# wagnva/semantic-nerf-for-satellite-data

Measured on AMD Instinct MI355X. Metric: train rays/sec (4096 rays x 64 samples), higher is better.
Workload: dtype f32(f16x2)

## Files before the change

semantic-nerf-for-satellite-data_amd/csrc/api.hip:

```cpp
#include <stdarg.h>
#include <stdio.h>
#include <stdlib.h>
#include <string.h>

#include <mutex>

#include "aux_kernels.h"
#include "bsp.h"
#include "composite.h"
#include "gemm.h"
#include "plan.h"

namespace snerf {

int forward_bsp(const Plan& p, const float* pk, const SnerfInputs* in, const SnerfOutputs* out, void* workspace, hipStream_t st);
int backward_bsp(const Plan& p, const float* pk, const SnerfInputs* in, const SnerfOutGrads* go, float* gp, float* d_t, float* d_t_s,
                 void* workspace, hipStream_t st);

static thread_local char g_err[512] = "";
void set_error(const char* fmt, ...) {
  va_list ap;
  va_start(ap, fmt);
  vsnprintf(g_err, sizeof(g_err), fmt, ap);
  va_end(ap);
// ... 359 lines not shown
  return p.packed_floats;
}

size_t snerf_grad_floats(const SnerfDesc* desc) {
  Plan p;
  if (make_plan(desc, &p)) return 0;
  return p.n_fp32;
}

size_t snerf_workspace_bytes(const SnerfDesc* desc) {
  Plan p;
  if (make_plan(desc, &p)) return 0;
  return p.ws_bytes;
}

int snerf_pack_params(const SnerfDesc* desc, const SnerfParams* params, float* packed, void* stream) {
  Plan p;
  RC(make_plan(desc, &p));
  if (!params || !packed) { set_error("null params/packed"); return SNERF_ERR_NULL; }
  TableBuilder tb;
  build_tables(p, params, tb);
  if (tb.missing) { set_error("snerf_pack_params: a parameter tensor required by this SnerfDesc is NULL"); return SNERF_ERR_NULL; }
  hipStream_t st = (hipStream_t)stream;
  RC(launch_zero_bytes(packed, p.n_fp32 * sizeof(float), st));
  for (int i = 0; i < tb.nt; ++i) RC(launch_copy_table(tb.tabs[i], packed, 0, st));
  char* planes = reinterpret_cast<char*>(packed + p.n_fp32);
  int* exps = reinterpret_cast<int*>(planes + p.wp_bytes);
  unsigned* maxbits = reinterpret_cast<unsigned*>(exps + bsp::WPACK_MAX);
  note_plan(packed, p.compose_feats);
  if (!p.compose_feats) return bsp::launch_wpack(p.wj, packed, planes, exps, maxbits, p.pl, st);
  {
    bsp::SgTable tb;
    bsp::compose_jobs(tb, packed + p.w_h1, packed + p.w_fs, packed + p.b_fs, packed + p.b_h1, packed + p.o_wc, packed + p.o_bc, p.W, p.FA, p.N1);
    RC(bsp::launch_sgemm(tb, 64, st));
  }
  bsp::WPackTable first, rest;
  first.n = rest.n = 0;
  for (int i = 0; i < p.wj.n; ++i) (i < p.wj_first ? first.j[first.n++] : rest.j[rest.n++]) = p.wj.j[i];
  RC(bsp::launch_wpack(first, packed, planes, exps, maxbits, p.pl, st));
  return bsp::launch_wpack(rest, packed, planes, exps, maxbits, p.pl, st);
}

int snerf_unpack_grads(const SnerfDesc* desc, const float* packed_grads, const SnerfParams* grads, int accumulate,
                       void* stream) {
  Plan p;
  RC(make_plan(desc, &p));
  if (!grads || !packed_grads) { set_error("null grads"); return SNERF_ERR_NULL; }
  TableBuilder tb;
  build_tables(p, grads, tb);
  if (tb.missing) { set_error("snerf_unpack_grads: a gradient tensor required by this SnerfDesc is NULL"); return SNERF_ERR_NULL; }
  hipStream_t st = (hipStream_t)stream;
  for (int i = 0; i < tb.nt; ++i) RC(launch_copy_table(tb.tabs[i], const_cast<float*>(packed_grads), accumulate ? 2 : 1, st));
  return SNERF_OK;
}

int snerf_forward(const SnerfDesc* desc, const float* packed_params, const SnerfInputs* in, const SnerfOutputs* out,
                  void* workspace, size_t workspace_bytes, void* stream) {
  Plan p;
  RC(make_plan(desc, &p));
  if (!packed_params || !out || !workspace) { set_error("snerf_forward: null argument"); return SNERF_ERR_NULL; }
  if (workspace_bytes < p.ws_bytes) { set_error("snerf_forward: workspace too small (%zu < %zu)", workspace_bytes, p.ws_bytes); return SNERF_ERR_WORKSPACE; }
  if (((uintptr_t)workspace & 255) || ((uintptr_t)packed_params & 255)) { set_error("workspace and packed params must be 256-byte aligned"); return SNERF_ERR_WORKSPACE; }
  RC(check_inputs(p, in));
  RC(check_plan_note(packed_params, p.compose_feats, "snerf_forward", "packed parameter buffer"));
  if (p.relight) {
    RC(check_plan_note(workspace, p.compose_feats, "snerf_forward", "workspace"));
    RC(check_relight_note(workspace, desc, out->beta != nullptr));
// ... 42 lines not shown
```

semantic-nerf-for-satellite-data_amd/csrc/bsp.h:

```cpp
#pragma once
#include "common.h"
#include "gemm.h"

namespace snerf {
namespace bsp {

constexpr int RB = 128;
constexpr int CB = 128;
constexpr int E_MAX = 100;
constexpr int E_QUIET = 60;

typedef __amdgpu_buffer_rsrc_t srd_t;
typedef unsigned int u32x4 __attribute__((ext_vector_type(4)));
typedef unsigned int u32x2 __attribute__((ext_vector_type(2)));
typedef _Float16 f16x8 __attribute__((ext_vector_type(8)));
typedef _Float16 f16x4 __attribute__((ext_vector_type(4)));
constexpr unsigned OOB = 0xFFFFFFF0u;

__host__ __device__ inline int ncb_of(int ld) { return (ld + CB - 1) / CB; }
__host__ __device__ inline size_t plane_bytes(size_t rows, int ld, int pl = 2) { return rows * (size_t)ld * 2 * pl; }
__host__ __device__ inline size_t etab_ints(size_t rows, int ld) { return ((rows + RB - 1) / RB) * (size_t)ncb_of(ld); }
__host__ __device__ inline unsigned g16_off(int k, int pl = 2) { return (unsigned)(k >> 4) * 32u * (unsigned)pl + (unsigned)(k & 15) * 2u; }

__host__ __device__ inline int exp_of_maxbits(unsigned b) {
// ... 127 lines not shown
bool trunk_fusion_enabled();

int launch_kc(const KcArgs& a, hipStream_t st);
void kc_set_grid_override(int n);
int launch_kc_narrow(const KcArgs& a, hipStream_t st);
int launch_dw(const DwArgs& a, bool narrow_i, hipStream_t st);

int launch_to_planes(const float* src, int ld_src, int rows, int cols, char* dst, int* E, int ld, int col0, int pl, hipStream_t st);
int launch_from_planes(const char* src, const int* E, int ld, int col0, int rows, int cols, float* dst, int ld_dst, int pl, hipStream_t st);

struct WPackJob {
  unsigned long long src_off;
  int src_ld;
  int rows, K;
  int transposed;
  unsigned long long dst_off;
  int e_idx;
  int m_rows, m_cols;
};
constexpr int WPACK_MAX = 48;
struct WPackTable { WPackJob j[WPACK_MAX]; int n; };
constexpr int WPACK_CHUNK = 24;
struct WPackChunk { WPackJob j[WPACK_CHUNK]; int n; };
__host__ __device__ inline size_t wp16_bytes(int rows, int K, int pl = 2) { return (size_t)((rows + 31) / 32) * (size_t)(K / 16) * 1024 * pl; }
int launch_wpack(const WPackTable& tb, const float* master, char* planes, int* exps, unsigned* maxbits, int pl, hipStream_t st);

struct SgJob {
  const float* A = nullptr; long long sa_i = 0, sa_k = 0;
  const float* B = nullptr; long long sb_k = 0, sb_j = 0;
  const float* D = nullptr; int ldd = 0;
  const float* u = nullptr; const float* v = nullptr;
  float* C = nullptr; int ldc = 0;
  int M = 0, N = 0, K = 0, acc = 0;
  int blk0 = 0;
};
constexpr int SG_MAX = 6;
struct SgTable { SgJob j[SG_MAX]; int n = 0; };
int launch_sgemm(const SgTable& tb, int tile_m, hipStream_t st);
void compose_jobs(SgTable& tb, const float* w_h1, const float* w_f, const float* b_f, const float* b_h1, float* wc, float* bc, int W, int FA, int N1);
void uncompose_jobs(SgTable& tb, const float* G, const float* gc, const float* w_h1, const float* w_f, const float* b_f,
                    float* dw_h1, float* db_h1, float* dw_f, float* db_f, int W, int FA, int M);

}
struct EncodeArgs;
namespace bsp {
int launch_encode_bsp(const EncodeArgs& a, char* pe, int* Epe, char* fa, int* Efa, int fa_col0, int pl, hipStream_t st);
int launch_relight_extras(const EncodeArgs& a, char* fa, int* Efa, int fa_col0, int pl, hipStream_t st);
int launch_zero_cols(char* base, size_t pitch, size_t width_bytes, int rows, hipStream_t st);
int launch_colsum32_bsp(const float* in, int rows, float* partial, char* planes, int* E, int pl, hipStream_t st);

}
}
```

semantic-nerf-for-satellite-data_amd/csrc/bsp_aux.hip:

```cpp
#include "bsp.h"
#include "aux_kernels.h"

namespace snerf {
namespace bsp {

__device__ __forceinline__ float block_max_256(float m, float* sm) {
#pragma unroll
  for (int o = 32; o >= 1; o >>= 1) m = fmaxf(m, __shfl_xor(m, o, 64));
  __syncthreads();
  if ((threadIdx.x & 63) == 0) sm[threadIdx.x >> 6] = m;
  __syncthreads();
  return fmaxf(fmaxf(sm[0], sm[1]), fmaxf(sm[2], sm[3]));
}

__global__ __launch_bounds__(256) void to_planes_kernel(const float* __restrict__ src, int ld_src, int rows, int cols,
                                                        char* __restrict__ dst, int* __restrict__ E, int ld, int col0, int pl) {
  __shared__ float sm[4];
  const int rb = blockIdx.y, cb = blockIdx.x;
  const int t = threadIdx.x, c8 = cb * 128 + (t & 15) * 8;
  float v[8][8];
  float m = 0.f;
#pragma unroll
  for (int i = 0; i < 8; ++i) {
    const int r = rb * 128 + (t >> 4) + 16 * i;
// ... 76 lines not shown
    const int r = threadIdx.x >> 3, kp = (threadIdx.x & 7) * 2;
    const int ra = ub * 32 + wf16_row(r), ka = ks * 16 + kp;
    float x[2];
#pragma unroll
    for (int q = 0; q < 2; ++q) {
      const int k = ka + q;
      const bool ok = j.transposed ? (k < j.m_rows && ra < j.m_cols) : (ra < j.m_rows && k < j.m_cols);
      x[q] = ok ? master[j.src_off + (j.transposed ? (size_t)k * j.src_ld + ra : (size_t)ra * j.src_ld + k)] : 0.f;
    }
    const _Float16 h0 = (_Float16)(x[0] * sc), h1 = (_Float16)(x[1] * sc);
    const _Float16 l0 = (_Float16)(x[0] * sc - (float)h0), l1 = (_Float16)(x[1] * sc - (float)h1);
    typedef _Float16 f16x2 __attribute__((ext_vector_type(2)));
    char* u = planes + j.dst_off + (size_t)unit * 1024 * pl + (32 * (kp >> 3) + r) * 16 + (kp & 7) * 2;
    *reinterpret_cast<f16x2*>(u) = f16x2{h0, h1};
    if (pl == 2) *reinterpret_cast<f16x2*>(u + 1024) = f16x2{l0, l1};
  }
}

int launch_wpack(const WPackTable& tb, const float* master, char* planes, int* exps, unsigned* maxbits, int pl, hipStream_t st) {
  if (tb.n <= 0) return SNERF_OK;
  { int rc = launch_zero_bytes(maxbits, WPACK_MAX * sizeof(unsigned), st); if (rc) return rc; }
  for (int pass = 0; pass < 2; ++pass)
    for (int first = 0; first < tb.n; first += WPACK_CHUNK) {
      WPackChunk c;
      c.n = tb.n - first < WPACK_CHUNK ? tb.n - first : WPACK_CHUNK;
      for (int i = 0; i < c.n; ++i) c.j[i] = tb.j[first + i];
      if (pass == 0) hipLaunchKernelGGL(wmax_kernel, dim3(32, c.n), dim3(256), 0, st, c, master, maxbits);
      else hipLaunchKernelGGL(wpack_kernel, dim3(128, c.n), dim3(256), 0, st, c, master, planes, exps, maxbits, pl);
      SNERF_LAUNCH_CHECK();
    }
  return SNERF_OK;
}

template <int TM>
__global__ __launch_bounds__(256) void sgemm_jobs_kernel(const SgTable tb) {
  constexpr int BM = 16 * TM, BN = 64, BK = 16;
  __shared__ float As[BK][BM + 1];
  __shared__ float Bs[BK][BN + 4];
  int q = 0;
  while (q + 1 < tb.n && (int)blockIdx.x >= tb.j[q + 1].blk0) ++q;
  const SgJob jb = tb.j[q];
  const int tiles_n = (jb.N + BN - 1) / BN;
  const int tile = (int)blockIdx.x - jb.blk0;
  const int i0 = (tile / tiles_n) * BM, j0 = (tile % tiles_n) * BN;
  const int t = threadIdx.x, ty = t >> 4, tx = t & 15;
  float acc[TM][4];
#pragma unroll
  for (int r = 0; r < TM; ++r)
#pragma unroll
    for (int c = 0; c < 4; ++c) acc[r][c] = 0.f;
  const bool a_k_fast = jb.sa_k == 1, b_j_fast = jb.sb_j == 1;
  for (int k0 = 0; k0 < jb.K; k0 += BK) {
#pragma unroll
    for (int s = 0; s < (BM * BK) / 256; ++s) {
      const int idx = t + 256 * s;
      const int i = a_k_fast ? idx / BK : idx % BM, k = a_k_fast ? idx % BK : idx / BM;
      As[k][i] = (i0 + i < jb.M && k0 + k < jb.K) ? jb.A[(long long)(i0 + i) * jb.sa_i + (long long)(k0 + k) * jb.sa_k] : 0.f;
    }
#pragma unroll
    for (int s = 0; s < (BN * BK) / 256; ++s) {
      const int idx = t + 256 * s;
      const int j = b_j_fast ? idx % BN : idx / BK, k = b_j_fast ? idx / BN : idx % BK;
      Bs[k][j] = (j0 + j < jb.N && k0 + k < jb.K) ? jb.B[(long long)(k0 + k) * jb.sb_k + (long long)(j0 + j) * jb.sb_j] : 0.f;
    }
    __syncthreads();
#pragma unroll
    for (int k = 0; k < BK; ++k) {
      float a[TM], b[4];
#pragma unroll
      for (int r = 0; r < TM; ++r) a[r] = As[k][ty * TM + r];
#pragma unroll
      for (int c = 0; c < 4; ++c) b[c] = Bs[k][tx * 4 + c];
#pragma unroll
      for (int r = 0; r < TM; ++r)
#pragma unroll
        for (int c = 0; c < 4; ++c) acc[r][c] = fmaf(a[r], b[c], acc[r][c]);
    }
    __syncthreads();
  }
#pragma unroll
  for (int r = 0; r < TM; ++r) {
    const int i = i0 + ty * TM + r;
    if (i >= jb.M) continue;
#pragma unroll
    for (int c = 0; c < 4; ++c) {
      const int j = j0 + tx * 4 + c;
      if (j >= jb.N) continue;
      float x = acc[r][c];
      if (jb.u) x = fmaf(jb.u[i], jb.v[j], x);
      if (jb.D) x += jb.D[(size_t)i * jb.ldd + j];
      float* o = jb.C + (size_t)i * jb.ldc + j;
      *o = jb.acc ? *o + x : x;
    }
  }
}

void compose_jobs(SgTable& tb, const float* w_h1, const float* w_f, const float* b_f, const float* b_h1, float* wc, float* bc, int W, int FA, int N1) {
  const int X = FA - W;
  tb.n = 0;
  auto job = [&]() -> SgJob& { tb.j[tb.n] = SgJob(); return tb.j[tb.n++]; };
  { SgJob& j = job(); j.A = w_h1; j.sa_i = FA; j.sa_k = 1; j.B = w_f; j.sb_k = W; j.sb_j = 1; j.C = wc; j.ldc = FA; j.M = N1; j.N = W; j.K = W; }
  { SgJob& j = job(); j.D = w_h1 + W; j.ldd = FA; j.C = wc + W; j.ldc = FA; j.M = N1; j.N = X; }
  { SgJob& j = job(); j.D = w_f + (size_t)W * W; j.ldd = W; j.C = wc + (size_t)N1 * FA; j.ldc = FA; j.M = 32; j.N = W; }
  { SgJob& j = job(); j.C = wc + (size_t)N1 * FA + W; j.ldc = FA; j.M = 32; j.N = X; }
  { SgJob& j = job(); j.A = w_h1; j.sa_i = FA; j.sa_k = 1; j.B = b_f; j.sb_k = 1; j.sb_j = 0; j.D = b_h1; j.ldd = 1; j.C = bc; j.ldc = 1; j.M = N1; j.N = 1; j.K = W; }
}
void uncompose_jobs(SgTable& tb, const float* G, const float* gc, const float* w_h1, const float* w_f, const float* b_f,
                    float* dw_h1, float* db_h1, float* dw_f, float* db_f, int W, int FA, int M) {
  tb.n = 0;
  auto job = [&]() -> SgJob& { tb.j[tb.n] = SgJob(); return tb.j[tb.n++]; };
  { SgJob& j = job(); j.A = G; j.sa_i = FA; j.sa_k = 1; j.B = w_f; j.sb_k = 1; j.sb_j = W; j.u = gc; j.v = b_f; j.C = dw_h1; j.ldc = FA; j.M = M; j.N = W; j.K = W; j.acc = 1; }
  { SgJob& j = job(); j.A = w_h1; j.sa_i = 1; j.sa_k = FA; j.B = G; j.sb_k = FA; j.sb_j = 1; j.C = dw_f; j.ldc = W; j.M = W; j.N = W; j.K = M; j.acc = 1; }
  { SgJob& j = job(); j.A = w_h1; j.sa_i = 1; j.sa_k = FA; j.B = gc; j.sb_k = 1; j.sb_j = 0; j.C = db_f; j.ldc = 1; j.M = W; j.N = 1; j.K = M; j.acc = 1; }
  { SgJob& j = job(); j.D = gc; j.ldd = 1; j.C = db_h1; j.ldc = 1; j.M = M; j.N = 1; j.acc = 1; }
}

int launch_sgemm(const SgTable& tb0, int tile_m, hipStream_t st) {
  if (tb0.n <= 0) return SNERF_OK;
  if (tb0.n > SG_MAX || (tile_m != 64 && tile_m != 32)) { set_error("sgemm: bad job table"); return SNERF_ERR_BAD_DESC; }
  SgTable tb = tb0;
  int blocks = 0;
  for (int q = 0; q < tb.n; ++q) {
    SgJob& j = tb.j[q];
    if (!j.C || j.M <= 0 || j.N <= 0 || j.K < 0 || j.ldc < 1 || (j.K > 0 && (!j.A || !j.B)) || (j.u && !j.v) || (j.D && j.ldd < 1)) {
      set_error("sgemm: bad job %d", q);
      return SNERF_ERR_BAD_DESC;
    }
    j.blk0 = blocks;
    blocks += ((j.M + tile_m - 1) / tile_m) * ((j.N + 63) / 64);
  }
  if (tile_m == 64) hipLaunchKernelGGL(sgemm_jobs_kernel<4>, dim3(blocks), dim3(256), 0, st, tb);
  else hipLaunchKernelGGL(sgemm_jobs_kernel<2>, dim3(blocks), dim3(256), 0, st, tb);
  SNERF_LAUNCH_CHECK();
  return SNERF_OK;
}

__global__ void zero_cols_kernel(char* base, size_t pitch, int width16, int rows) {
  const int i = blockIdx.x * blockDim.x + threadIdx.x;
  if (i >= rows * width16) return;
  const int r = i / width16, c = i - r * width16;
  *reinterpret_cast<u32x4*>(base + (size_t)r * pitch + 16 * (size_t)c) = u32x4{0u, 0u, 0u, 0u};
}
int launch_zero_cols(char* base, size_t pitch, size_t width_bytes, int rows, hipStream_t st) {
  const int w16 = (int)(width_bytes / 16);
  if (w16 <= 0 || rows <= 0) return SNERF_OK;
  hipLaunchKernelGGL(zero_cols_kernel, dim3((unsigned)(((size_t)rows * w16 + 255) / 256)), dim3(256), 0, st, base, pitch, w16, rows);
  SNERF_LAUNCH_CHECK();
  return SNERF_OK;
}

__device__ __forceinline__ void point_xyz(const EncodeArgs& a, long long point, float (&x)[3]) {
  const int n = (int)((unsigned)point / (unsigned)a.S);
#pragma unroll
  for (int c = 0; c < 3; ++c) {
    if (a.xyz != nullptr) {
      x[c] = a.xyz[point * 3 + c];
    } else {
#pragma clang fp contract(off)
      const float o = a.rays[n * 8 + c];
      const float d = a.dir_is_sun ? a.sun_d[(size_t)n * a.sun_stride + c] : a.rays[n * 8 + 3 + c];
      const float dz = d * a.z[point];
      x[c] = o + dz;
    }
  }
}
// ... 197 lines not shown
```

semantic-nerf-for-satellite-data_amd/csrc/bsp_gemm.hip:

```cpp
#include "bsp_dev.h"

#include <vector>

namespace snerf {
namespace bsp {

constexpr int KC_STRIP = 32 * 68 * 4;
constexpr int KN_A = 128 * 64, KN_RING = 4, KN_TAIL = KN_RING * KN_A, KN_LDS = KN_TAIL + 512;

template <int PL>
__global__ __launch_bounds__(256, 4) void gemm_kcn_kernel(const KcArgs p) {
  constexpr int EB = 2 * PL, KSUB = PL == 2 ? 16 : 32, KSH = PL == 2 ? 4 : 5;
  __shared__ __attribute__((aligned(16))) char lds[KN_LDS];
  int* etab = reinterpret_cast<int*>(lds + KN_TAIL);
  const int t = threadIdx.x, lane = t & 63;
  const int wave = __builtin_amdgcn_readfirstlane(t >> 6);
  const int ti = blockIdx.x, i0 = ti * 128, wi0 = wave * 32;
  const int nks16 = p.K >> 4;
  const int nks = (p.K + KSUB - 1) >> KSH, nks1 = nks;
  const srd_t srdA = make_srd(p.A + ((size_t)i0 * p.lda + p.a_col0) * EB,
                              clamp_bytes(i0 < p.I ? ((unsigned long long)(p.I - i0 - 1) * p.lda + p.Ka) * (unsigned long long)EB : 0ull));
  const srd_t srdW = make_srd(p.W, p.w_bytes);
  unsigned voA[2];
#pragma unroll
  for (int q = 0; q < 2; ++q) {
    const int row = 64 * q + (t >> 2);
    const unsigned c = (unsigned)((t & 3) ^ ((row >> 2) & 3));
    voA[q] = (i0 + row < p.I) ? (unsigned)row * (unsigned)p.lda * (unsigned)EB + 16u * c : OOB;
  }
  const unsigned w_u0 = (unsigned)(p.w_row0 >> 5), w_ks0 = (unsigned)(p.w_k0 >> 4);
  auto issueA = [&](int s, int slot) {
#pragma unroll
    for (int q = 0; q < 2; ++q) dma16(srdA, lds + slot * KN_A + 4096 * q + wave * 1024, s < nks ? voA[q] : OOB, (unsigned)s * 64u);
  };
// ... 29 lines not shown
  const unsigned fo0 = (unsigned)rowl * 64u + (unsigned)(((0 + kh) ^ swz) << 4);
  const unsigned fo1 = (unsigned)rowl * 64u + (unsigned)(((2 + kh) ^ swz) << 4);
  auto step = [&](int s, int slot, BFrag& bc, BFrag& bn) {
    wait_vm<2>();
    barrier_raw();
    if (__builtin_expect(((s < 64 ? chg0 >> s : chg1 >> (s - 64)) & 1ull) != 0ull, 0)) acc = scale_acc(acc, etab[s] - etab[s - 1]);
    loadB(s + 1, bn);
    issueA(s + 2, (slot + 2) % KN_RING);
    const char* st = lds + slot * KN_A;
    if constexpr (PL == 2) {
      acc = mfma3(ldsfrag(st + wi0 * 64 + fo0), ldsfrag(st + wi0 * 64 + fo1), __builtin_bit_cast(f16x8, bc.h), __builtin_bit_cast(f16x8, bc.l), acc);
    } else {
      acc = __builtin_amdgcn_mfma_f32_32x32x16_f16(ldsfrag(st + wi0 * 64 + fo0), __builtin_bit_cast(f16x8, bc.h), acc, 0, 0, 0);
      acc = __builtin_amdgcn_mfma_f32_32x32x16_f16(ldsfrag(st + wi0 * 64 + fo1), __builtin_bit_cast(f16x8, bc.l), acc, 0, 0, 0);
    }
  };
  for (int s = 0; s < nks; s += 4) {
    step(s, 0, bq0, bq1);
    if (s + 1 < nks) step(s + 1, 1, bq1, bq0);
    if (s + 2 < nks) step(s + 2, 2, bq0, bq1);
    if (s + 3 < nks) step(s + 3, 3, bq1, bq0);
  }
  wait_vm<0>();
  const int e_in = e_last + *p.EW;
  const int col = wf16_row(lane & 31);
  const float bj = (p.bias != nullptr && col < p.J) ? p.bias[col] : 0.f;
#pragma unroll
  for (int r = 0; r < 16; ++r) {
    const int row = i0 + wi0 + (r & 3) + 8 * (r >> 2) + 4 * (lane >> 5);
    if (row < p.I && col < p.J) p.Cf[(size_t)row * 32 + col] = __builtin_amdgcn_ldexpf(acc[r], -e_in) + bj;
  }
}

template <int TI, int PL> struct DwCfg {
  static constexpr int NTH = TI == 256 ? 512 : 256, WAVES = NTH / 64;
  static constexpr int MI = TI == 256 ? 4 : 1;
  static constexpr int EB = 2 * PL;
  static constexpr int PTS = PL == 2 ? 16 : 32;
  static constexpr int SPC = 128 / PTS;
  static constexpr int A_PITCH = TI * EB;
  static constexpr int B_PITCH = 256 * EB;
  static constexpr int A_BYTES = PTS * A_PITCH, B_BYTES = PTS * B_PITCH, STAGE = A_BYTES + B_BYTES, RING = 3;
  static constexpr int STRIPS = WAVES * KC_STRIP;
  static constexpr int TAIL = (RING * STAGE > STRIPS) ? RING * STAGE : STRIPS;
  static constexpr int MAXCH = 128;
  static constexpr int DUMMY = TAIL + WAVES * MAXCH * 4;
  static constexpr int LDS = DUMMY + (TI == 256 ? 0 : WAVES * 1024);
};
template <int PITCH> __device__ __forceinline__ unsigned dw_swz(int p) {
  return PITCH == 1024 ? (unsigned)(((p & 1) << 5) | ((p & 2) << 6)) : (PITCH == 512 ? (unsigned)((p & 3) << 6) : (PITCH == 128 ? (unsigned)((p & 2) << 4) : 0u));
}

template <int TI, int PL>
__global__ __launch_bounds__(TI == 256 ? 512 : 256, 2) void gemm_dw_kernel(const DwArgs p) {
  using T = DwCfg<TI, PL>;
  constexpr int EB = T::EB, PTS = T::PTS;
  __shared__ __attribute__((aligned(16))) char lds[T::LDS];
  int* esum = reinterpret_cast<int*>(lds + T::TAIL);

  const int t = threadIdx.x, lane = t & 63;
  const int wave = __builtin_amdgcn_readfirstlane(t >> 6);
  const int wi0 = TI == 256 ? (wave >> 2) * 128 : 0, wj0 = (wave & 3) * 64;
  int tile, split;
  split_tile_of_block(blockIdx.x, blockIdx.z, gridDim.x, gridDim.z, tile, split);
  const int ti = tile / p.tiles_j, tj = tile - ti * p.tiles_j;
  const int i0 = ti * TI, j0 = tj * 256;
  const int kBeg = split * p.k_split, kEnd = min(p.P, kBeg + p.k_split);
  const int nks = (kEnd - kBeg + PTS - 1) / PTS;
  float* C = p.C + (size_t)split * p.slab_stride;

  const srd_words srdA = make_srd_words(p.A + ((size_t)kBeg * p.lda + p.a_col0 + i0) * EB,
                                        clamp_bytes(kEnd > kBeg ? ((unsigned long long)(kEnd - kBeg) * p.lda - (p.a_col0 + i0)) * (unsigned long long)EB : 0ull));
  const srd_words srdB = make_srd_words(p.B + ((size_t)kBeg * p.ldb + p.b_col0 + j0) * EB,
                                        clamp_bytes(kEnd > kBeg ? ((unsigned long long)(kEnd - kBeg) * p.ldb - (p.b_col0 + j0)) * (unsigned long long)EB : 0ull));
  const unsigned lds0 = __builtin_amdgcn_readfirstlane(lds_addr(lds));
  constexpr int PA = T::A_PITCH, PB = T::B_PITCH;
  constexpr int A_PIECES = T::A_BYTES / 1024;
  constexpr int NPA = (A_PIECES + T::WAVES - 1) / T::WAVES;
  constexpr int NPB = 16 / T::WAVES;
  constexpr int RPA = PA >= 1024 ? 1 : 1024 / PA, RPB = 1024 / PB;
  constexpr int LRA = 64 / RPA, LRB = 64 / RPB;
  unsigned voA[NPA], voB[NPB];
  int prA[NPA], prB[NPB];
#pragma unroll
  for (int q = 0; q < NPA; ++q) {
    const int piece = wave * NPA + q;
    const int pr = piece * RPA + lane / LRA;
    const unsigned byte = 16u * (unsigned)(lane % LRA);
    prA[q] = piece < A_PIECES ? pr : -1;
    voA[q] = (unsigned)pr * (unsigned)p.lda * (unsigned)EB + (byte ^ dw_swz<PA>(pr));
  }
#pragma unroll
  for (int q = 0; q < NPB; ++q) {
    const int piece = wave * NPB + q;
    const int pr = piece * RPB + lane / LRB;
    prB[q] = pr;
    voB[q] = (unsigned)pr * (unsigned)p.ldb * (unsigned)EB + ((16u * (unsigned)(lane % LRB)) ^ dw_swz<PB>(pr));
  }
  auto issue = [&](int s, int slot) {
    const int prow0 = kBeg + PTS * s;
#pragma unroll
    for (int q = 0; q < NPA; ++q) {
      const int piece = wave * NPA + q;
      const bool ok = s < nks && prA[q] >= 0 && prow0 + prA[q] < kEnd;
      dma16_asm(srdA, lds0 + (unsigned)(piece < A_PIECES ? slot * T::STAGE + piece * 1024 : T::DUMMY + wave * 1024), ok ? voA[q] : OOB,
                (unsigned)s * (unsigned)PTS * (unsigned)p.lda * (unsigned)EB);
    }
#pragma unroll
    for (int q = 0; q < NPB; ++q) {
      const bool ok = s < nks && prow0 + prB[q] < kEnd;
      dma16_asm(srdB, lds0 + (unsigned)(slot * T::STAGE + T::A_BYTES + (wave * NPB + q) * 1024), ok ? voB[q] : OOB, (unsigned)s * (unsigned)PTS * (unsigned)p.ldb * (unsigned)EB);
    }
  };
  const int nch = (kEnd - kBeg + 127) >> 7;
  {
    const int ncbA = ncb_of(p.lda), ncbB = ncb_of(p.ldb);
    const int cbA = min((p.a_col0 + i0 + wi0) >> 7, ncbA - 1), cbB = min((p.b_col0 + j0 + wj0) >> 7, ncbB - 1);
    for (int c = lane; c < nch; c += 64) {
      const size_t rb = (size_t)(kBeg >> 7) + c;
      esum[wave * T::MAXCH + c] = p.EA[rb * ncbA + cbA] + p.EB[rb * ncbB + cbB];
    }
  }

  issue(0, 0);
  issue(1, 1);
#pragma unroll
  for (int r = 2; r < T::RING - 1; ++r) issue(r, r);

  f32x16 acc[T::MI][2];
#pragma unroll
  for (int mi = 0; mi < T::MI; ++mi)
#pragma unroll
    for (int nj = 0; nj < 2; ++nj)
#pragma unroll
      for (int r = 0; r < 16; ++r) acc[mi][nj][r] = 0.f;

  const int g = lane >> 4, q4 = (lane >> 2) & 3, pp = lane & 3;
  const int kq = 8 * (g >> 1) + q4;
  auto frag_off = [&](int col, int pl, int pitch, unsigned sw) -> unsigned {
    if constexpr (PL == 2) return (unsigned)kq * (unsigned)pitch + ((((unsigned)(col >> 4) * 64u) + (unsigned)pl * 32u + 8u * (unsigned)pp) ^ sw);
    else return (unsigned)(kq + 16 * pl) * (unsigned)pitch + ((((unsigned)(col >> 4) * 32u) + 8u * (unsigned)pp) ^ sw);
  };
  unsigned foA[T::MI][2], foB[2][2];
#pragma unroll
  for (int mi = 0; mi < T::MI; ++mi)
#pragma unroll
    for (int pl = 0; pl < 2; ++pl) foA[mi][pl] = frag_off(wi0 + 32 * mi + 16 * (g & 1), pl, PA, dw_swz<PA>(q4));
#pragma unroll
  for (int nj = 0; nj < 2; ++nj)
#pragma unroll
    for (int pl = 0; pl < 2; ++pl) foB[nj][pl] = (unsigned)T::A_BYTES + frag_off(wj0 + 32 * nj + 16 * (g & 1), pl, PB, dw_swz<PB>(q4));
  typedef __fp16 h4_t __attribute__((__vector_size__(4 * sizeof(__fp16))));
  typedef h4_t __attribute__((address_space(3))) * lds4_t;
  auto trfrag = [&](const char* base, unsigned off, int pitch) -> f16x8 {
    const f16x4 a = __builtin_bit_cast(f16x4, __builtin_amdgcn_ds_read_tr16_b64_v4f16((lds4_t)(base + off)));
    const f16x4 b = __builtin_bit_cast(f16x4, __builtin_amdgcn_ds_read_tr16_b64_v4f16((lds4_t)(base + off + 4 * pitch)));
    return f16x8{a[0], a[1], a[2], a[3], b[0], b[1], b[2], b[3]};
  };

  int e_cur = 0;
  bool quiet = false;
  constexpr int NPIECE = NPA + NPB;
  auto mma = [](f16x8 ah, f16x8 al, f16x8 bh, f16x8 bl, f32x16 c) -> f32x16 {
    if constexpr (PL == 2) return mfma3(ah, al, bh, bl, c);
    c = __builtin_amdgcn_mfma_f32_32x32x16_f16(ah, bh, c, 0, 0, 0);
    return __builtin_amdgcn_mfma_f32_32x32x16_f16(al, bl, c, 0, 0, 0);
  };
  auto chunk = [&](int s) {
    if ((s & (T::SPC - 1)) != 0) return;
    const int e_new = __builtin_amdgcn_readfirstlane(esum[wave * T::MAXCH + s / T::SPC]);
    quiet = s != 0 && e_new - e_cur > 64;
    if (s == 0) e_cur = e_new;
    else if (__builtin_expect(e_new != e_cur && !quiet, 0)) {
      const int de = e_new - e_cur;
#pragma unroll
      for (int mi = 0; mi < T::MI; ++mi)
#pragma unroll
        for (int nj = 0; nj < 2; ++nj) acc[mi][nj] = scale_acc(acc[mi][nj], de);
      e_cur = e_new;
    }
  };
  const bool active = (j0 + wj0 < p.J) && (i0 + wi0 < p.I);
  if constexpr (TI == 256) {
    const int grp = wave >> 2;
    f16x8 fa_h[4], fa_l[4], fb_h[2], fb_l[2];
    auto phaseM = [&](int s, int slot) {
      issue(s + T::RING - 1, (slot + T::RING - 1) % T::RING);
      if (!active) return;
      chunk(s);
      const char* st = lds + slot * T::STAGE;
#pragma unroll
      for (int nj = 0; nj < 2; ++nj) { fb_h[nj] = trfrag(st, foB[nj][0], PB); fb_l[nj] = trfrag(st, foB[nj][1], PB); }
#pragma unroll
      for (int mi = 0; mi < 4; ++mi) { fa_h[mi] = trfrag(st, foA[mi][0], PA); fa_l[mi] = trfrag(st, foA[mi][1], PA); }
      if (__builtin_expect(quiet, 0)) {
#pragma unroll
        for (int nj = 0; nj < 2; ++nj) { fb_h[nj] = f16x8{}; fb_l[nj] = f16x8{}; }
      }
    };
    auto phaseC = [&]() {
      if (!active) return;
      __builtin_amdgcn_s_setprio(1);
#pragma unroll
      for (int mi = 0; mi < 4; ++mi)
#pragma unroll
        for (int nj = 0; nj < 2; ++nj) acc[mi][nj] = mma(fa_h[mi], fa_l[mi], fb_h[nj], fb_l[nj], acc[mi][nj]);
      __builtin_amdgcn_s_setprio(0);
    };
    wait_vm<(T::RING - 2) * NPIECE>();
    barrier_raw();
    if (grp == 0) {
      int slot = 0;
      for (int s = 0; s < nks; ++s) {
        phaseM(s, slot);
        barrier_raw();
        phaseC();
        wait_vm<(T::RING - 2) * NPIECE>();
        barrier_raw();
        slot = slot == T::RING - 1 ? 0 : slot + 1;
      }
      barrier_raw();
    } else {
      barrier_raw();
      int slot = 0;
      for (int s = 0; s < nks; ++s) {
        phaseM(s, slot);
        wait_vm<(T::RING - 2) * NPIECE>();
        barrier_raw();
        phaseC();
        barrier_raw();
        slot = slot == T::RING - 1 ? 0 : slot + 1;
      }
    }
  } else
  {
  auto step = [&](int s, int slot) {
    wait_vm<NPIECE>();
// ... 75 lines not shown
    return SNERF_OK;
  }
  if (!a.C || !a.EC || (a.ldc & 15) || (a.c_col0 & 127) || (a.J & 15) || a.c_col0 + a.J > a.ldc) return bad("BSP output: ldc % 16, c_col0 % 128, J % 16");
  if (((uintptr_t)a.C & 15) || (a.bias && ((uintptr_t)a.bias & 15))) return bad("output / bias alignment");
  if (a.aux_mode != AUX_NONE) {
    if (a.aux_mode != AUX_SINREC && a.aux_mode != AUX_RELU_MASK) return bad("unsupported aux mode");
    if (!a.H || !a.EH || (a.ldh & 15) || (a.h_col0 & 127) || a.h_col0 + a.J > a.ldh) return bad("aux tensor: ldh % 16, h_col0 % 128");
    if (a.aux_mode == AUX_SINREC && !a.Hsign) return bad("AUX_SINREC needs the sign words");
    if (a.act != ACT_NONE) return bad("activation and derivative in one epilogue");
  }
  if (a.colsum && (((uintptr_t)a.colsum & 15) || (a.ldcs & 3))) return bad("colsum alignment");
  if (a.nd_w != nullptr) {
    if (a.act != ACT_SIN || a.aux_mode != AUX_NONE || !a.nd_out || (a.J & 255) || a.J > 2048 || a.nd_stride < (unsigned long long)a.I || ((uintptr_t)a.nd_w & 15))
      return bad("folded projection: ACT_SIN forward launch of whole 256-column tiles, J <= 2048, nd_out [tiles_j * 4 * nd_omax][nd_stride >= I]");
  }
  if ((size_t)128 * a.ldc * EB >= 0x7FFFFFFFull) return bad("ldc too large");
  return SNERF_OK;
}

int launch_kc_narrow(const KcArgs& a0, hipStream_t st) {
  KcArgs a = a0;
  if (a.Ka == 0) a.Ka = a.K;
  a.A2 = a.A; a.EA2 = a.EA; a.lda2 = a.lda; a.a2_col0 = a.a_col0;
  int rc = check_kc(a, true);
  if (rc) return rc;
  const int tok = prof_hook_begin(2.0 * a.I * 32.0 * a.K, 3, st);
  if (a.pl == 2) hipLaunchKernelGGL(gemm_kcn_kernel<2>, dim3((a.I + 127) / 128), dim3(256), 0, st, a);
  else hipLaunchKernelGGL(gemm_kcn_kernel<1>, dim3((a.I + 127) / 128), dim3(256), 0, st, a);
  SNERF_LAUNCH_CHECK();
  prof_hook_end(tok, st);
  return SNERF_OK;
}

int launch_dw(const DwArgs& a0, bool narrow_i, hipStream_t st) {
  DwArgs a = a0;
  if (!a.A || !a.EA || !a.B || !a.EB || !a.C) return bad("dW: null operand");
  if (a.I <= 0 || a.J <= 0 || a.P <= 0) return bad("dW: empty problem");
  if ((a.lda & 15) || (a.ldb & 15) || (a.a_col0 & 15) || (a.b_col0 & 15) || (a.J & 3) || (a.ldc & 3)) return bad("dW: leading dimensions / column offsets");
  if (a.k_split <= 0 || (a.k_split & 127) || a.k_split > 16384 || a.n_split < 1) return bad("dW: k_split must be a multiple of 128, <= 16384");
  if (a.pl != 1 && a.pl != 2) return bad("dW: planes: 1 or 2");
  if ((size_t)a.k_split * (a.lda > a.ldb ? a.lda : a.ldb) * 2 * a.pl >= 0xFFFFFFF0ull) return bad("dW: k_split * ld exceeds the 32-bit span");
  if (narrow_i ? (a.I > 32 || ((a.a_col0 & 127) + 32 > 128)) : ((a.a_col0 & 127) != 0)) return bad("dW: the A columns of a wave must lie in one exponent block");
  if (a.b_col0 & 63) return bad("dW: b_col0 % 64");
  if (((uintptr_t)a.A & 15) || ((uintptr_t)a.B & 15) || ((uintptr_t)a.C & 15)) return bad("dW: alignment");
  const int TI = narrow_i ? 32 : 256;
  a.tiles_i = (a.I + TI - 1) / TI;
  a.tiles_j = (a.J + 255) / 256;
  const dim3 grid(a.tiles_i * a.tiles_j, 1, a.n_split);
  const int tok = prof_hook_begin(2.0 * a.I * (double)a.J * a.P, narrow_i ? 3 : 2, st);
  if (narrow_i) { if (a.pl == 2) hipLaunchKernelGGL((gemm_dw_kernel<32, 2>), grid, dim3(256), 0, st, a); else hipLaunchKernelGGL((gemm_dw_kernel<32, 1>), grid, dim3(256), 0, st, a); }
  else { if (a.pl == 2) hipLaunchKernelGGL((gemm_dw_kernel<256, 2>), grid, dim3(512), 0, st, a); else hipLaunchKernelGGL((gemm_dw_kernel<256, 1>), grid, dim3(512), 0, st, a); }
  SNERF_LAUNCH_CHECK();
  prof_hook_end(tok, st);
  return SNERF_OK;
}

}
}
```

semantic-nerf-for-satellite-data_amd/csrc/bsp_pass.hip:

```cpp
#include "aux_kernels.h"
#include "bsp.h"
#include "composite.h"
#include "plan.h"

namespace snerf {

namespace {
struct Ws {
  char* base;
  char* c(size_t off) const { return base + off; }
  float* f(size_t off) const { return reinterpret_cast<float*>(base + off); }
  int* i(size_t off) const { return reinterpret_cast<int*>(base + off); }
  unsigned* u(size_t off) const { return reinterpret_cast<unsigned*>(base + off); }
  void a(bsp::KcArgs& g, const PlaneT& t, int k, int col0 = 0) const { g.A = c(t.o); g.EA = i(t.e); g.lda = t.ld; g.a_col0 = col0; g.Ka = k; }
  void a2(bsp::KcArgs& g, const PlaneT& t) const { g.A2 = c(t.o); g.EA2 = i(t.e); g.lda2 = t.ld; }
  void out(bsp::KcArgs& g, const PlaneT& t, int col0 = 0) const { g.C = c(t.o); g.EC = i(t.e); g.ldc = t.ld; g.c_col0 = col0; g.Csign = t.s ? u(t.s) : nullptr; }
  void h(bsp::KcArgs& g, const PlaneT& t, int col0 = 0) const { g.H = c(t.o); g.EH = i(t.e); g.ldh = t.ld; g.h_col0 = col0; g.Hsign = t.s ? u(t.s) : nullptr; }
  void dz(bsp::DwArgs& g, const PlaneT& t) const { g.A = c(t.o); g.EA = i(t.e); g.lda = t.ld; g.a_col0 = 0; }
  void x(bsp::DwArgs& g, const PlaneT& t, int col0) const { g.B = c(t.o); g.EB = i(t.e); g.ldb = t.ld; g.b_col0 = col0; }
};
struct WOp { const char* W; const int* EW; int rb32; unsigned bytes; int K; };
WOp wop(const Plan& p, const float* pk, int job) {
  const char* planes = reinterpret_cast<const char*>(pk + p.n_fp32);
  const bsp::WPackJob& w = p.wj.j[job];
// ... 389 lines not shown
    colsum(g, r.cs_hl, W);
    RC(launch_kc(g));
    RC(bias_from_colsum(r.cs_hl, W, gp + p.b_tr[p.L - 1]));
  }
  for (int i = p.L - 1; i >= 0; --i) {
    const BwdRegions::Layer& t = r.tr[i];
    if (i > 0 && ((p.skip_mask >> i) & 1u)) {
      RC(dw_gemm(t.w_gamma, dz_cur, W, false, p.pe, 0, p.Ep));
      RC(dw_gemm(t.w, dz_cur, W, false, p.h[i - 1], 0, W));
      RC(red_add_elem2d(rq.elem, t.w_gamma.slab, t.w_gamma.sp.ns, t.w_gamma.stride, W, p.Ep, p.Ep, gp + p.w_tr[i], p.k_tr[i]));
      RC(red_add_elem2d(rq.elem, t.w.slab, t.w.sp.ns, t.w.stride, W, W, W, gp + p.w_tr[i] + p.Ep, p.k_tr[i]));
    } else {
      if (i == 0) RC(dw_gemm(t.w, dz_cur, W, false, p.pe, 0, p.Ep));
      else RC(dw_gemm(t.w, dz_cur, W, false, p.h[i - 1], 0, W));
      RC(dw_reduce(t.w, (size_t)W * p.k_tr[i], gp + p.w_tr[i]));
    }
    if (i == 0) break;
    bsp::KcArgs g;
    ws.a(g, dz_cur, W); weights(g, p, pk, p.wj_tt[i]);
    g.I = P; g.J = W; g.K = W; ws.out(g, dz_nxt);
    dact(g, p.h[i - 1], 0, (i - 1 == 0) ? 30.f : 1.f);
    colsum(g, t.cs, W);
    RC(launch_kc(g));
    RC(bias_from_colsum(t.cs, W, gp + p.b_tr[i - 1]));
    const PlaneT sw = dz_cur; dz_cur = dz_nxt; dz_nxt = sw;
  }
  RC(launch_reductions(rq.elem, rq.col, st));
  if (!uncompose) return SNERF_OK;
  {
    const size_t r0 = p.sc ? (size_t)p.sun_col : 0;
    bsp::SgTable tb;
    bsp::uncompose_jobs(tb, r.w_h1.slab, r.cs_fin, pk + p.w_h1 + r0 * p.FA, pk + p.w_fs, pk + p.b_fs,
                        gp + p.w_h1 + r0 * p.FA, gp + p.b_h1 + r0, gp + p.w_fs, gp + p.b_fs, W, p.FA, p.h1w);
    return bsp::launch_sgemm(tb, 32, st);
  }
}

}
```

Measured before the change: 165,000.

## Rewrite job-table SGEMM with double-buffered square tiles and add thin-J dW kernel

Replaces the small FP32 job-table SGEMM with a version that uses square 32 or 64 tiles chosen per job by job size, a larger K block, register-prefetched double-buffered LDS and vector fragment loads, so compose and uncompose GEMMs overlap loads with FMAs. It also adds a gemm_dw_kernel variant with a 64-wide J tile for weight-gradient GEMMs where J<=64, avoiding wasted work in 256-wide tiles. The new thin variant is on by default and can be disabled with an environment variable. Risks are new indexing and swizzle paths for the thin tile, and higher register and LDS use in the SGEMM.

After: 166,600 (median of 6 runs). Within noise of the previous version (+1.0%).

```diff
diff --git a/semantic-nerf-for-satellite-data_amd/csrc/api.hip b/semantic-nerf-for-satellite-data_amd/csrc/api.hip
--- a/semantic-nerf-for-satellite-data_amd/csrc/api.hip
+++ b/semantic-nerf-for-satellite-data_amd/csrc/api.hip
@@ -415,7 +415,7 @@
   {
     bsp::SgTable tb;
     bsp::compose_jobs(tb, packed + p.w_h1, packed + p.w_fs, packed + p.b_fs, packed + p.b_h1, packed + p.o_wc, packed + p.o_bc, p.W, p.FA, p.N1);
-    RC(bsp::launch_sgemm(tb, 64, st));
+    RC(bsp::launch_sgemm(tb, st));
   }
   bsp::WPackTable first, rest;
   first.n = rest.n = 0;
diff --git a/semantic-nerf-for-satellite-data_amd/csrc/bsp.h b/semantic-nerf-for-satellite-data_amd/csrc/bsp.h
--- a/semantic-nerf-for-satellite-data_amd/csrc/bsp.h
+++ b/semantic-nerf-for-satellite-data_amd/csrc/bsp.h
@@ -183,11 +183,11 @@
   const float* u = nullptr; const float* v = nullptr;
   float* C = nullptr; int ldc = 0;
   int M = 0, N = 0, K = 0, acc = 0;
-  int blk0 = 0;
+  int blk0 = 0, tile = 0;
 };
 constexpr int SG_MAX = 6;
 struct SgTable { SgJob j[SG_MAX]; int n = 0; };
-int launch_sgemm(const SgTable& tb, int tile_m, hipStream_t st);
+int launch_sgemm(const SgTable& tb, hipStream_t st);
 void compose_jobs(SgTable& tb, const float* w_h1, const float* w_f, const float* b_f, const float* b_h1, float* wc, float* bc, int W, int FA, int N1);
 void uncompose_jobs(SgTable& tb, const float* G, const float* gc, const float* w_h1, const float* w_f, const float* b_f,
                     float* dw_h1, float* db_h1, float* dw_f, float* db_f, int W, int FA, int M);
diff --git a/semantic-nerf-for-satellite-data_amd/csrc/bsp_aux.hip b/semantic-nerf-for-satellite-data_amd/csrc/bsp_aux.hip
--- a/semantic-nerf-for-satellite-data_amd/csrc/bsp_aux.hip
+++ b/semantic-nerf-for-satellite-data_amd/csrc/bsp_aux.hip
@@ -132,67 +132,132 @@
   return SNERF_OK;
 }
 
+constexpr int SG_BK = 32;
+constexpr int SG_LDS_FLOATS = 2 * 2 * SG_BK * (64 + 4);
+
 template <int TM>
+__device__ __forceinline__ void sgemm_tile(const SgJob& jb, int tile, float* __restrict__ sm) {
+  constexpr int BT = 16 * TM, BK = SG_BK, LD = BT + 4, NL = (BT * BK) / 256;
+  float* As = sm;
+  float* Bs = sm + 2 * BK * LD;
+  const int tiles_n = (jb.N + BT - 1) / BT;
+  const int i0 = (tile / tiles_n) * BT, j0 = (tile % tiles_n) * BT;
+  const int t = threadIdx.x, ty = t >> 4, tx = t & 15;
+  const bool a_k_fast = jb.sa_k == 1, b_j_fast = jb.sb_j == 1;
+  float acc[TM][TM];
+#pragma unroll
+  for (int r = 0; r < TM; ++r)
+#pragma unroll
+    for (int c = 0; c < TM; ++c) acc[r][c] = 0.f;
+  auto coord = [&](int s, bool row_fast, int& row, int& k) {
+    const int idx = t + 256 * s;
+    if (row_fast) { row = idx % BT; k = idx / BT; }
+    else { row = (idx >> 4) % BT; k = (idx & 15) + 16 * ((idx >> 4) / BT); }
+  };
+  float xa[NL], xb[NL];
+  auto fetch = [&](int k0) {
+#pragma unroll
+    for (int s = 0; s < NL; ++s) {
+      int i, k;
+      coord(s, !a_k_fast, i, k);
+      xa[s] = jb.A[(long long)min(i0 + i, jb.M - 1) * jb.sa_i + (long long)min(k0 + k, jb.K - 1) * jb.sa_k];
+    }
+#pragma unroll
+    for (int s = 0; s < NL; ++s) {
+      int j, k;
+      coord(s, b_j_fast, j, k);
+      xb[s] = jb.B[(long long)min(k0 + k, jb.K - 1) * jb.sb_k + (long long)min(j0 + j, jb.N - 1) * jb.sb_j];
+    }
+  };
+  auto stash = [&](int k0, int buf) {
+#pragma unroll
+    for (int s = 0; s < NL; ++s) {
+      int i, j, k;
+      coord(s, !a_k_fast, i, k);
+      As[(buf * BK + k) * LD + i] = (i0 + i < jb.M && k0 + k < jb.K) ? xa[s] : 0.f;
+      coord(s, b_j_fast, j, k);
+      Bs[(buf * BK + k) * LD + j] = (j0 + j < jb.N && k0 + k < jb.K) ? xb[s] : 0.f;
+    }
+  };
+  constexpr int KU = 4;
+  typedef float fragv __attribute__((ext_vector_type(TM)));
+  auto contract = [&](int buf) {
+    const float* as = As + buf * BK * LD + ty * TM;
+    const float* bs = Bs + buf * BK * LD + tx * TM;
+    fragv af[2][KU], bf[2][KU];
+    auto frags = [&](int g, int k) {
+#pragma unroll
+      for (int u = 0; u < KU; ++u) {
+        af[g][u] = *reinterpret_cast<const fragv*>(as + (k + u) * LD);
+        bf[g][u] = *reinterpret_cast<const fragv*>(bs + (k + u) * LD);
+      }
+    };
+    auto fmas = [&](int g) {
+#pragma unroll
+      for (int u = 0; u < KU; ++u)
+#pragma unroll
+        for (int r = 0; r < TM; ++r)
+#pragma unroll
+          for (int c = 0; c < TM; ++c) acc[r][c] = fmaf(af[g][u][r], bf[g][u][c], acc[r][c]);
+    };
+    frags(0, 0);
+#pragma unroll 1
+    for (int k = 0; k < BK; k += 2 * KU) {
+      frags(1, k + KU);
+      fmas(0);
+      if (k + 2 * KU < BK) frags(0, k + 2 * KU);
+      fmas(1);
+    }
+  };
+  const int nk = (jb.K + BK - 1) / BK;
+  if (nk > 0) {
+    fetch(0);
+    stash(0, 0);
+    __syncthreads();
+  }
+  for (int n = 0; n < nk; ++n) {
+    const bool more = n + 1 < nk;
+    if (more) fetch((n + 1) * BK);
+    contract(n & 1);
+    if (more) stash((n + 1) * BK, (n + 1) & 1);
+    __syncthreads();
+  }
+  int ic[TM], jc[TM];
+#pragma unroll
+  for (int r = 0; r < TM; ++r) { ic[r] = min(i0 + ty * TM + r, jb.M - 1); jc[r] = min(j0 + tx * TM + r, jb.N - 1); }
+  float uu[TM], vv[TM], dd[TM][TM], oo[TM][TM];
+#pragma unroll
+  for (int r = 0; r < TM; ++r) {
+    uu[r] = jb.u ? jb.u[ic[r]] : 0.f;
+    vv[r] = jb.u ? jb.v[jc[r]] : 0.f;
+#pragma unroll
+    for (int c = 0; c < TM; ++c) {
+      dd[r][c] = jb.D ? jb.D[(size_t)ic[r] * jb.ldd + jc[c]] : 0.f;
+      oo[r][c] = jb.acc ? jb.C[(size_t)ic[r] * jb.ldc + jc[c]] : 0.f;
+    }
+  }
+#pragma unroll
+  for (int r = 0; r < TM; ++r) {
+    const int i = i0 + ty * TM + r;
+#pragma unroll
+    for (int c = 0; c < TM; ++c) {
+      const int j = j0 + tx * TM + c;
+      float x = acc[r][c];
+      if (jb.u) x = fmaf(uu[r], vv[c], x);
+      if (jb.D) x += dd[r][c];
+      if (i < jb.M && j < jb.N) jb.C[(size_t)i * jb.ldc + j] = jb.acc ? oo[r][c] + x : x;
+    }
+  }
+}
+
 __global__ __launch_bounds__(256) void sgemm_jobs_kernel(const SgTable tb) {
-  constexpr int BM = 16 * TM, BN = 64, BK = 16;
-  __shared__ float As[BK][BM + 1];
-  __shared__ float Bs[BK][BN + 4];
+  __shared__ __attribute__((aligned(16))) float sm[SG_LDS_FLOATS];
   int q = 0;
   while (q + 1 < tb.n && (int)blockIdx.x >= tb.j[q + 1].blk0) ++q;
   const SgJob jb = tb.j[q];
-  const int tiles_n = (jb.N + BN - 1) / BN;
-  const int tile = (int)blockIdx.x - jb.blk0;
-  const int i0 = (tile / tiles_n) * BM, j0 = (tile % tiles_n) * BN;
-  const int t = threadIdx.x, ty = t >> 4, tx = t & 15;
-  float acc[TM][4];
-#pragma unroll
-  for (int r = 0; r < TM; ++r)
-#pragma unroll
-    for (int c = 0; c < 4; ++c) acc[r][c] = 0.f;
-  const bool a_k_fast = jb.sa_k == 1, b_j_fast = jb.sb_j == 1;
-  for (int k0 = 0; k0 < jb.K; k0 += BK) {
-#pragma unroll
-    for (int s = 0; s < (BM * BK) / 256; ++s) {
-      const int idx = t + 256 * s;
-      const int i = a_k_fast ? idx / BK : idx % BM, k = a_k_fast ? idx % BK : idx / BM;
-      As[k][i] = (i0 + i < jb.M && k0 + k < jb.K) ? jb.A[(long long)(i0 + i) * jb.sa_i + (long long)(k0 + k) * jb.sa_k] : 0.f;
-    }
-#pragma unroll
-    for (int s = 0; s < (BN * BK) / 256; ++s) {
-      const int idx = t + 256 * s;
-      const int j = b_j_fast ? idx % BN : idx / BK, k = b_j_fast ? idx / BN : idx % BK;
-      Bs[k][j] = (j0 + j < jb.N && k0 + k < jb.K) ? jb.B[(long long)(k0 + k) * jb.sb_k + (long long)(j0 + j) * jb.sb_j] : 0.f;
-    }
-    __syncthreads();
-#pragma unroll
-    for (int k = 0; k < BK; ++k) {
-      float a[TM], b[4];
-#pragma unroll
-      for (int r = 0; r < TM; ++r) a[r] = As[k][ty * TM + r];
-#pragma unroll
-      for (int c = 0; c < 4; ++c) b[c] = Bs[k][tx * 4 + c];
-#pragma unroll
-      for (int r = 0; r < TM; ++r)
-#pragma unroll
-        for (int c = 0; c < 4; ++c) acc[r][c] = fmaf(a[r], b[c], acc[r][c]);
-    }
-    __syncthreads();
-  }
-#pragma unroll
-  for (int r = 0; r < TM; ++r) {
-    const int i = i0 + ty * TM + r;
-    if (i >= jb.M) continue;
-#pragma unroll
-    for (int c = 0; c < 4; ++c) {
-      const int j = j0 + tx * 4 + c;
-      if (j >= jb.N) continue;
-      float x = acc[r][c];
-      if (jb.u) x = fmaf(jb.u[i], jb.v[j], x);
-      if (jb.D) x += jb.D[(size_t)i * jb.ldd + j];
-      float* o = jb.C + (size_t)i * jb.ldc + j;
-      *o = jb.acc ? *o + x : x;
-    }
-  }
+  const int tile =(int)blockIdx.x - jb.blk0;
+  if (jb.tile == 64) sgemm_tile<4>(jb, tile, sm);
+  else sgemm_tile<2>(jb, tile, sm);
 }
 
 void compose_jobs(SgTable& tb, const float* w_h1, const float* w_f, const float* b_f, const float* b_h1, float* wc, float* bc, int W, int FA, int N1) {
@@ -215,9 +280,10 @@
   { SgJob& j = job(); j.D = gc; j.ldd = 1; j.C = db_h1; j.ldc = 1; j.M = M; j.N = 1; j.acc = 1; }
 }
 
-int launch_sgemm(const SgTable& tb0, int tile_m, hipStream_t st) {
+constexpr int SG_WIDE_MIN = 128;
+int launch_sgemm(const SgTable& tb0, hipStream_t st) {
   if (tb0.n <= 0) return SNERF_OK;
-  if (tb0.n > SG_MAX || (tile_m != 64 && tile_m != 32)) { set_error("sgemm: bad job table"); return SNERF_ERR_BAD_DESC; }
+  if (tb0.n > SG_MAX) { set_error("sgemm: bad job table"); return SNERF_ERR_BAD_DESC; }
   SgTable tb = tb0;
   int blocks = 0;
   for (int q = 0; q < tb.n; ++q) {
@@ -226,11 +292,14 @@
       set_error("sgemm: bad job %d", q);
       return SNERF_ERR_BAD_DESC;
     }
+    const long long wide = (long long)((j.M + 63) / 64) * ((j.N + 63) / 64);
+    j.tile = wide >= SG_WIDE_MIN ? 64 : 32;
     j.blk0 = blocks;
-    blocks += ((j.M + tile_m - 1) / tile_m) * ((j.N + 63) / 64);
-  }
-  if (tile_m == 64) hipLaunchKernelGGL(sgemm_jobs_kernel<4>, dim3(blocks), dim3(256), 0, st, tb);
-  else hipLaunchKernelGGL(sgemm_jobs_kernel<2>, dim3(blocks), dim3(256), 0, st, tb);
+    const long long nb = (long long)((j.M + j.tile - 1) / j.tile) * ((j.N + j.tile - 1) / j.tile);
+    if (nb + blocks > (1 << 24)) { set_error("sgemm: job %d too large", q); return SNERF_ERR_BAD_DESC; }
+    blocks += (int)nb;
+  }
+  hipLaunchKernelGGL(sgemm_jobs_kernel, dim3(blocks), dim3(256), 0, st, tb);
   SNERF_LAUNCH_CHECK();
   return SNERF_OK;
 }
diff --git a/semantic-nerf-for-satellite-data_amd/csrc/bsp_gemm.hip b/semantic-nerf-for-satellite-data_amd/csrc/bsp_gemm.hip
--- a/semantic-nerf-for-satellite-data_amd/csrc/bsp_gemm.hip
+++ b/semantic-nerf-for-satellite-data_amd/csrc/bsp_gemm.hip
@@ -1,5 +1,6 @@
 #include "bsp_dev.h"
 
+#include <cstdlib>
 #include <vector>
 
 namespace snerf {
@@ -95,35 +96,38 @@
   }
 }
 
-template <int TI, int PL> struct DwCfg {
+template <int TI, int PL, int TJ = 256> struct DwCfg {
   static constexpr int NTH = TI == 256 ? 512 : 256, WAVES = NTH / 64;
-  static constexpr int MI = TI == 256 ? 4 : 1;
+  static constexpr int MI = (TI == 256 && TJ == 256) ? 4 : 1;
   static constexpr int EB = 2 * PL;
   static constexpr int PTS = PL == 2 ? 16 : 32;
   static constexpr int SPC = 128 / PTS;
   static constexpr int A_PITCH = TI * EB;
-  static constexpr int B_PITCH = 256 * EB;
+  static constexpr int B_PITCH = TJ * EB;
   static constexpr int A_BYTES = PTS * A_PITCH, B_BYTES = PTS * B_PITCH, STAGE = A_BYTES + B_BYTES, RING = 3;
   static constexpr int STRIPS = WAVES * KC_STRIP;
   static constexpr int TAIL = (RING * STAGE > STRIPS) ? RING * STAGE : STRIPS;
   static constexpr int MAXCH = 128;
   static constexpr int DUMMY = TAIL + WAVES * MAXCH * 4;
-  static constexpr int LDS = DUMMY + (TI == 256 ? 0 : WAVES * 1024);
+  static constexpr int LDS = DUMMY + (TI == 256 ? (TJ == 256 ? 0 : 4 * 1024) : WAVES * 1024);
 };
-template <int PITCH> __device__ __forceinline__ unsigned dw_swz(int p) {
-  return PITCH == 1024 ? (unsigned)(((p & 1) << 5) | ((p & 2) << 6)) : (PITCH == 512 ? (unsigned)((p & 3) << 6) : (PITCH == 128 ? (unsigned)((p & 2) << 4) : 0u));
-}
-
-template <int TI, int PL>
+template <int PITCH, int PL> __device__ __forceinline__ unsigned dw_swz(int p) {
+  if (PITCH == 1024 || PITCH == 256) return (unsigned)(((p & 1) << 5) | ((p & 2) << 6));
+  if (PITCH == 512) return (unsigned)((p & 3) << 6);
+  if (PITCH == 128) return PL == 2 ? (unsigned)((p & 2) << 4) : (unsigned)((p & 2) << 5);
+  return 0u;
+}
+
+template <int TI, int PL, int TJ = 256>
 __global__ __launch_bounds__(TI == 256 ? 512 : 256, 2) void gemm_dw_kernel(const DwArgs p) {
-  using T = DwCfg<TI, PL>;
+  using T = DwCfg<TI, PL, TJ>;
   constexpr int EB = T::EB, PTS = T::PTS;
   __shared__ __attribute__((aligned(16))) char lds[T::LDS];
   int* esum = reinterpret_cast<int*>(lds + T::TAIL);
 
   const int t = threadIdx.x, lane = t & 63;
   const int wave = __builtin_amdgcn_readfirstlane(t >> 6);
-  const int wi0 = TI == 256 ? (wave >> 2) * 128 : 0, wj0 = (wave & 3) * 64;
+  const int wi0 = TJ == 64 ? wave * 32 : (TI == 256 ? (wave >> 2) * 128 : 0), wj0 = TJ == 64 ? 0 : (wave & 3) * 64;
   int tile, split;
   split_tile_of_block(blockIdx.x, blockIdx.z, gridDim.x, gridDim.z, tile, split);
   const int ti = tile / p.tiles_j, tj = tile - ti * p.tiles_j;
@@ -140,7 +144,8 @@
   constexpr int PA = T::A_PITCH, PB = T::B_PITCH;
   constexpr int A_PIECES = T::A_BYTES / 1024;
   constexpr int NPA = (A_PIECES + T::WAVES - 1) / T::WAVES;
-  constexpr int NPB = 16 / T::WAVES;
+  constexpr int B_PIECES = T::B_BYTES / 1024;
+  constexpr int NPB = (B_PIECES + T::WAVES - 1) / T::WAVES;
   constexpr int RPA = PA >= 1024 ? 1 : 1024 / PA, RPB = 1024 / PB;
   constexpr int LRA = 64 / RPA, LRB = 64 / RPB;
   unsigned voA[NPA], voB[NPB];
@@ -151,14 +156,14 @@
     const int pr = piece * RPA + lane / LRA;
     const unsigned byte = 16u * (unsigned)(lane % LRA);
     prA[q] = piece < A_PIECES ? pr : -1;
-    voA[q] = (unsigned)pr * (unsigned)p.lda * (unsigned)EB + (byte ^ dw_swz<PA>(pr));
+    voA[q] = (unsigned)pr * (unsigned)p.lda * (unsigned)EB + (byte ^ dw_swz<PA, PL>(pr));
   }
 #pragma unroll
   for (int q = 0; q < NPB; ++q) {
     const int piece = wave * NPB + q;
     const int pr = piece * RPB + lane / LRB;
-    prB[q] = pr;
-    voB[q] = (unsigned)pr * (unsigned)p.ldb * (unsigned)EB + ((16u * (unsigned)(lane % LRB)) ^ dw_swz<PB>(pr));
+    prB[q] = piece < B_PIECES ? pr : -1;
+    voB[q] = (unsigned)pr * (unsigned)p.ldb * (unsigned)EB + ((16u * (unsigned)(lane % LRB)) ^ dw_swz<PB, PL>(pr));
   }
   auto issue = [&](int s, int slot) {
     const int prow0 = kBeg + PTS * s;
@@ -171,8 +176,10 @@
     }
 #pragma unroll
     for (int q = 0; q < NPB; ++q) {
-      const bool ok = s < nks && prow0 + prB[q] < kEnd;
-      dma16_asm(srdB, lds0 + (unsigned)(slot * T::STAGE + T::A_BYTES + (wave * NPB + q) * 1024), ok ? voB[q] : OOB, (unsigned)s * (unsigned)PTS * (unsigned)p.ldb * (unsigned)EB);
+      const int piece = wave * NPB + q;
+      const bool ok = s < nks && prB[q] >= 0 && prow0 + prB[q] < kEnd;
+      dma16_asm(srdB, lds0 + (unsigned)(piece < B_PIECES ? slot * T::STAGE + T::A_BYTES + piece * 1024 : T::DUMMY + (wave & 3) * 1024), ok ? voB[q] : OOB,
+                (unsigned)s * (unsigned)PTS * (unsigned)p.ldb * (unsigned)EB);
     }
   };
   const int nch = (kEnd - kBeg + 127) >> 7;
@@ -208,11 +215,11 @@
 #pragma unroll
   for (int mi = 0; mi < T::MI; ++mi)
 #pragma unroll
-    for (int pl = 0; pl < 2; ++pl) foA[mi][pl] = frag_off(wi0 + 32 * mi + 16 * (g & 1), pl, PA, dw_swz<PA>(q4));
+    for (int pl = 0; pl < 2; ++pl) foA[mi][pl] = frag_off(wi0 + 32 * mi + 16 * (g & 1), pl, PA, dw_swz<PA, PL>(q4));
 #pragma unroll
   for (int nj = 0; nj < 2; ++nj)
 #pragma unroll
-    for (int pl = 0; pl < 2; ++pl) foB[nj][pl] = (unsigned)T::A_BYTES + frag_off(wj0 + 32 * nj + 16 * (g & 1), pl, PB, dw_swz<PB>(q4));
+    for (int pl = 0; pl < 2; ++pl) foB[nj][pl] = (unsigned)T::A_BYTES + frag_off(wj0 + 32 * nj + 16 * (g & 1), pl, PB, dw_swz<PB, PL>(q4));
   typedef __fp16 h4_t __attribute__((__vector_size__(4 * sizeof(__fp16))));
   typedef h4_t __attribute__((address_space(3))) * lds4_t;
   auto trfrag = [&](const char* base, unsigned off, int pitch) -> f16x8 {
@@ -246,7 +253,7 @@
   const bool active = (j0 + wj0 < p.J) && (i0 + wi0 < p.I);
   if constexpr (TI == 256) {
     const int grp = wave >> 2;
-    f16x8 fa_h[4], fa_l[4], fb_h[2], fb_l[2];
+    f16x8 fa_h[T::MI], fa_l[T::MI], fb_h[2], fb_l[2];
     auto phaseM = [&](int s, int slot) {
       issue(s + T::RING - 1, (slot + T::RING - 1) % T::RING);
       if (!active) return;
@@ -255,7 +262,7 @@
 #pragma unroll
       for (int nj = 0; nj < 2; ++nj) { fb_h[nj] = trfrag(st, foB[nj][0], PB); fb_l[nj] = trfrag(st, foB[nj][1], PB); }
 #pragma unroll
-      for (int mi = 0; mi < 4; ++mi) { fa_h[mi] = trfrag(st, foA[mi][0], PA); fa_l[mi] = trfrag(st, foA[mi][1], PA); }
+      for (int mi = 0; mi < T::MI; ++mi) { fa_h[mi] = trfrag(st, foA[mi][0], PA); fa_l[mi] = trfrag(st, foA[mi][1], PA); }
       if (__builtin_expect(quiet, 0)) {
 #pragma unroll
         for (int nj = 0; nj < 2; ++nj) { fb_h[nj] = f16x8{}; fb_l[nj] = f16x8{}; }
@@ -265,7 +272,7 @@
       if (!active) return;
       __builtin_amdgcn_s_setprio(1);
 #pragma unroll
-      for (int mi = 0; mi < 4; ++mi)
+      for (int mi = 0; mi < T::MI; ++mi)
 #pragma unroll
         for (int nj = 0; nj < 2; ++nj) acc[mi][nj] = mma(fa_h[mi], fa_l[mi], fb_h[nj], fb_l[nj], acc[mi][nj]);
       __builtin_amdgcn_s_setprio(0);
@@ -407,6 +414,11 @@
   return SNERF_OK;
 }
 
+static bool dw_thin_on() {
+  const char* e = getenv("SNERF_DW_THIN");
+  return !(e && e[0] == '0');
+}
+
 int launch_dw(const DwArgs& a0, bool narrow_i, hipStream_t st) {
   DwArgs a = a0;
   if (!a.A || !a.EA || !a.B || !a.EB || !a.C) return bad("dW: null operand");
@@ -423,7 +435,8 @@
   a.tiles_j = (a.J + 255) / 256;
   const dim3 grid(a.tiles_i * a.tiles_j, 1, a.n_split);
   const int tok = prof_hook_begin(2.0 * a.I * (double)a.J * a.P, narrow_i ? 3 : 2, st);
-  if (narrow_i) { if (a.pl == 2) hipLaunchKernelGGL((gemm_dw_kernel<32, 2>), grid, dim3(256), 0, st, a); else hipLaunchKernelGGL((gemm_dw_kernel<32, 1>), grid, dim3(256), 0, st, a); }
+  if (!narrow_i && a.J <= 64 && dw_thin_on()) { if (a.pl == 2) hipLaunchKernelGGL((gemm_dw_kernel<256, 2, 64>), grid, dim3(512), 0, st, a); else hipLaunchKernelGGL((gemm_dw_kernel<256, 1, 64>), grid, dim3(512), 0, st, a); }
+  else if (narrow_i) { if (a.pl == 2) hipLaunchKernelGGL((gemm_dw_kernel<32, 2>), grid, dim3(256), 0, st, a); else hipLaunchKernelGGL((gemm_dw_kernel<32, 1>), grid, dim3(256), 0, st, a); }
   else { if (a.pl == 2) hipLaunchKernelGGL((gemm_dw_kernel<256, 2>), grid, dim3(512), 0, st, a); else hipLaunchKernelGGL((gemm_dw_kernel<256, 1>), grid, dim3(512), 0, st, a); }
   SNERF_LAUNCH_CHECK();
   prof_hook_end(tok, st);
diff --git a/semantic-nerf-for-satellite-data_amd/csrc/bsp_pass.hip b/semantic-nerf-for-satellite-data_amd/csrc/bsp_pass.hip
--- a/semantic-nerf-for-satellite-data_amd/csrc/bsp_pass.hip
+++ b/semantic-nerf-for-satellite-data_amd/csrc/bsp_pass.hip
@@ -445,8 +445,8 @@
     bsp::SgTable tb;
     bsp::uncompose_jobs(tb, r.w_h1.slab, r.cs_fin, pk + p.w_h1 + r0 * p.FA, pk + p.w_fs, pk + p.b_fs,
                         gp + p.w_h1 + r0 * p.FA, gp + p.b_h1 + r0, gp + p.w_fs, gp + p.b_fs, W, p.FA, p.h1w);
-    return bsp::launch_sgemm(tb, 32, st);
-  }
-}
-
-}
+    return bsp::launch_sgemm(tb, st);
+  }
+}
+
+}
```
